# azmyrajab/polars_ols

Hardware: AMD Instinct MI355X
Metric: group_regressions_per_sec (higher is better)
Workload: dtype f32

## Files before the change

### polars_ols_amd/csrc/k4x_inverse.hip

```cpp
#include "k4_rolling.hpp"

namespace pols {

constexpr int KX_MAX = 128;

template <typename T>
struct XCtx {
    const K4Args &a;
    int64_t s;
    int first_chunk;
    int K, LD, NS, tid;
    double *P, *xs, *v, *bv, *beta, *red;
    const T *mycol;
    __device__ XCtx(const K4Args &a_, int64_t s_, int fc, double *lds) : a(a_), s(s_), first_chunk(fc) {
        K = a.k; LD = K | 1; NS = K * K + K; tid = threadIdx.x;
        P = lds; xs = P + (size_t)K * LD; v = xs + KX_MAX + 2; bv = v + KX_MAX; beta = bv + KX_MAX; red = beta + KX_MAX;
        mycol = tid < K ? static_cast<const T *>(a.xtab ? a.xtab[tid] : a.x[tid]) : static_cast<const T *>(a.y);
    }
    static __host__ __device__ size_t lds_doubles(int K) { return (size_t)K * (K | 1) + 4 * KX_MAX + 2 + 16; }

    __device__ __forceinline__ bool valid(int64_t i) const { return a.valid ? a.valid[s + i] != 0 : true; }
    __device__ __forceinline__ int64_t cnt(int64_t i) const { return a.cnt ? (int64_t)a.cnt[s + i] : i + 1; }
    __device__ __forceinline__ int64_t vidx(int64_t r) const { return a.vidx ? (int64_t)a.vidx[s + r] : r; }

    __device__ __forceinline__ void load_row(int64_t i) const {
        __syncthreads();
        if (tid <= K) xs[tid] = (double)mycol[s + i];
        __syncthreads();
    }
    __device__ double block_sum(double x) const {
        const double w = wave_sum_row3(x);
        __syncthreads();
        if ((tid & 63) == 63) red[tid >> 6] = w;
        __syncthreads();
        return red[0] + red[1] + red[2] + red[3];
    }
    __device__ void zero() const {
        for (int q = tid; q < K * LD; q += 256) P[q] = 0.0;
        if (tid < K) bv[tid] = 0.0;
        __syncthreads();
    }
    __device__ void gram_axpy(const double *src, double sign) const {
        for (int q = tid; q < K * K; q += 256) { const int i = q / K, c = q - i * K; P[i * LD + c] += sign * src[q]; }
        if (tid < K) bv[tid] += sign * src[K * K + tid];
        __syncthreads();
    }
    __device__ void gram_add_row(int64_t i, double sign) const {
        load_row(i);
        for (int q = tid; q < K * K; q += 256) { const int r = q / K, c = q - r * K; P[r * LD + c] += sign * (xs[r] * xs[c]); }
        if (tid < K) bv[tid] += sign * (xs[tid] * xs[K]);
        __syncthreads();
    }
    __device__ void gram_prefix(int64_t i, double sign, int nacc) const {
        if (i < 0) return;
        const int64_t c = i / a.chunk_len;
        gram_axpy(a.totals + (size_t)(first_chunk + c) * nacc, sign);
        for (int64_t j = c * a.chunk_len; j <= i; ++j)
            if (valid(j)) gram_add_row(j, sign);
    }
    __device__ void invert(double alpha) const {
        if (tid < K) P[tid * LD + tid] += alpha;
        __syncthreads();
        for (int j = 0; j < K; ++j) {
            const double p = 1.0 / P[j * LD + j];
            if (tid < K) v[tid] = P[tid * LD + j];
            __syncthreads();
            for (int q = tid; q < K * K; q += 256) {
                const int i = q / K, c = q - i * K;
                double val;
                if (i == j && c == j) val = -p;
                else if (i == j) val = v[c] * p;
                else if (c == j) val = v[i] * p;
                else val = P[i * LD + c] - v[i] * v[c] * p;
                P[i * LD + c] = val;
            }
            __syncthreads();
        }
        for (int q = tid; q < K * K; q += 256) { const int i = q / K, c = q - i * K; P[i * LD + c] = -P[i * LD + c]; }
        __syncthreads();
    }
    __device__ void matvec(const double *x, double *out) const {
        if (tid < K) {
            double acc = 0.0;
            const double *row = P + tid * LD;
            for (int c = 0; c < K; ++c) acc += row[c] * x[c];
            out[tid] = acc;
        }
        __syncthreads();
    }
    __device__ void rank1(double coef) const {
        for (int q = tid; q < K * K; q += 256) { const int i = q / K, c = q - i * K; P[i * LD + c] += coef * (v[i] * v[c]); }
        __syncthreads();
    }
    __device__ void sm_update(double sign) const {
        matvec(xs, v);
        const double xv = block_sum(tid < K ? xs[tid] * v[tid] : 0.0);
        rank1(-sign / (1.0 + sign * xv));
        if (tid < K) bv[tid] += sign * (xs[tid] * xs[K]);
        __syncthreads();
    }
    __device__ void solve_beta() const { matvec(bv, beta); }
    __device__ void store(int64_t i, bool have, T *coef, T *pred) const {
        const int64_t row = s + i;
        const double qnan = __longlong_as_double(0x7ff8000000000000LL);
        if (coef && tid < K) coef[row * K + tid] = (T)(have ? beta[tid] : qnan);
        if (pred) {
            load_row(i);
            const double p = block_sum(tid < K ? xs[tid] * (have ? beta[tid] : qnan) : 0.0);
            if (tid == 0) pred[row] = (T)p;
        }
    }
};

template <typename T, bool RLS>
__global__ void __launch_bounds__(256) kx_totals_kernel(const K4Args a) {
    extern __shared__ double lds[];
    const int64_t c = blockIdx.x;
    const K4Chunk ch = a.chunks[c];
    const K4Group G = a.groups[ch.group];
    XCtx<T> cx(a, G.start, G.first_chunk, lds);
    const int K = cx.K, nacc = cx.NS + (RLS ? 1 : 0);
    cx.zero();
    double decay = 1.0;
    for (int64_t i = ch.t0 - G.start; i < ch.t1 - G.start; ++i)
        if (cx.valid(i)) {
            if (RLS) {
                for (int q = cx.tid; q < K * cx.LD; q += 256) cx.P[q] *= a.ff;
                if (cx.tid < K) cx.bv[cx.tid] *= a.ff;
                decay *= a.ff;
                __syncthreads();
            }
            cx.gram_add_row(i, 1.0);
        }
    double *out = a.totals + (size_t)c * nacc;
    for (int q = cx.tid; q < K * K; q += 256) { const int i = q / K, cc = q - i * K; out[q] = cx.P[i * cx.LD + cc]; }
    if (cx.tid < K) out[K * K + cx.tid] = cx.bv[cx.tid];
    if (RLS && cx.tid == 0) out[cx.NS] = decay;
}

template <typename T>
__global__ void __launch_bounds__(256) kx_rolling_walk_kernel(const K4Args a) {
    extern __shared__ double lds[];
    const int64_t c = blockIdx.x;
    const K4Chunk ch = a.chunks[c];
    const K4Group G = a.groups[ch.group];
    XCtx<T> cx(a, G.start, G.first_chunk, lds);
    const int K = cx.K, nacc = cx.NS;
    const int64_t rel0 = ch.t0 - G.start, rel1 = ch.t1 - G.start;
    const int64_t w = a.window, mpv = G.mpv;
    const bool drop = a.drop_mode != 0;
    T *coef = static_cast<T *>(a.coef);
    T *pred = static_cast<T *>(a.pred);
    const double qnan = __longlong_as_double(0x7ff8000000000000LL);

    if (G.all_nan) {
        for (int64_t i = rel0; i < rel1; ++i) {
            if (coef && cx.tid < K) coef[(G.start + i) * K + cx.tid] = (T)qnan;
            if (pred && cx.tid == 0) pred[G.start + i] = (T)qnan;
        }
        return;
    }
    const int64_t j_min = drop ? 0 : max(mpv - w, (int64_t)0);
    const int64_t c0 = drop ? cx.cnt(mpv - 1) : 0;
    const bool longwarm = drop && c0 > w;
    auto old_of = [&](int64_t i) -> int64_t {
        if (!drop) return i - w;
        const int64_t R = cx.cnt(i) - 1;
        const int64_t r = (longwarm && R - c0 < w) ? R - c0 : R - w;
        return r < 0 ? -1 : cx.vidx(r);
    };
    auto gate = [&](int64_t i) -> bool {
        const int64_t i_start = i >= w ? i - w : 0;
        return cx.cnt(i) - cx.cnt(i_start) >= G.gate_n;
    };
    auto gram_state_at = [&](int64_t i) {
        cx.zero();
        cx.gram_prefix(i, 1.0, nacc);
        const int64_t o = (i >= 0) ? old_of(i) : -1;
        if (o >= j_min && i >= mpv) {
            cx.gram_prefix(o, -1.0, nacc);
            cx.gram_prefix(j_min - 1, 1.0, nacc);
        }
        if (longwarm && i >= mpv && cx.cnt(i) - 1 - c0 >= w) {
            cx.gram_prefix(cx.vidx(c0 - 1), 1.0, nacc);
            cx.gram_prefix(cx.vidx(w - 1), -1.0, nacc);
        }
    };

    bool inverted = false, have = false;
    int64_t prev_old = (rel0 > 0 && rel0 - 1 >= mpv) ? old_of(rel0 - 1) : -1;
    if (rel0 >= mpv && rel0 > 0) {
        int64_t ip = rel0 - 1;
        if (!(drop || ip == mpv - 1 || gate(ip))) {
            for (ip = rel0 - 2; ip >= mpv - 1; --ip)
                if (ip == mpv - 1 || gate(ip)) break;
        }
        gram_state_at(ip);
        cx.invert(a.alpha);
        cx.solve_beta();
        have = true;
        if (ip != rel0 - 1) {
            gram_state_at(rel0 - 1);
            cx.invert(a.alpha);
        }
        inverted = true;
    } else {
        gram_state_at(rel0 - 1);
    }
    for (int64_t i = rel0; i < rel1; ++i) {
        const bool vld = cx.valid(i);
        if (vld) {
            if (inverted) { cx.load_row(i); cx.sm_update(1.0); }
            else cx.gram_add_row(i, 1.0);
        }
        if (i >= mpv && (vld || !drop)) {
            const int64_t no = old_of(i);
            bool sub = false;
            if (drop) sub = (no != prev_old && no >= 0);
            else sub = (no >= j_min && no >= 0 && cx.valid(no));
            if (sub) { cx.load_row(no); cx.sm_update(-1.0); }
            prev_old = no;
        }
        if (i >= mpv - 1) {
            const bool do_solve = (i == mpv - 1) || (drop ? vld : gate(i));
            if (do_solve) {
                if (!inverted) { cx.invert(a.alpha); inverted = true; }
                cx.solve_beta();
                have = true;
            }
        }
        cx.store(i, have, coef, pred);
    }
}

template <typename T>
__global__ void __launch_bounds__(256) kx_rls_walk_kernel(const K4Args a) {
    extern __shared__ double lds[];
    const int64_t c = blockIdx.x;
    const K4Chunk ch = a.chunks[c];
    const K4Group G = a.groups[ch.group];
    XCtx<T> cx(a, G.start, G.first_chunk, lds);
    const int K = cx.K, nacc = cx.NS + 1;
    const int64_t rel0 = ch.t0 - G.start, rel1 = ch.t1 - G.start;
    T *coef = static_cast<T *>(a.coef);
    T *pred = static_cast<T *>(a.pred);
    cx.zero();
    cx.gram_axpy(a.totals + (size_t)c * nacc, 1.0);
    cx.invert(0.0);
    cx.solve_beta();
    const double ff = a.ff;
    for (int64_t i = rel0; i < rel1; ++i) {
        if (cx.valid(i)) {
            cx.load_row(i);
            cx.matvec(cx.xs, cx.v);
            const double xv = cx.block_sum(cx.tid < K ? cx.xs[cx.tid] * cx.v[cx.tid] : 0.0);
            const double xb = cx.block_sum(cx.tid < K ? cx.xs[cx.tid] * cx.beta[cx.tid] : 0.0);
            const double r = 1.0 + xv / ff;
            const double err = cx.xs[K] - xb;
            if (cx.tid < K) cx.beta[cx.tid] += cx.v[cx.tid] / (r * ff) * err;
            const double coef_vv = -1.0 / (r * ff);
            for (int q = cx.tid; q < K * K; q += 256) {
                const int ii = q / K, cc = q - ii * K;
                cx.P[ii * cx.LD + cc] = (cx.P[ii * cx.LD + cc] + coef_vv * (cx.v[ii] * cx.v[cc])) / ff;
            }
            __syncthreads();
        }
        cx.store(i, true, coef, pred);
    }
}

template <typename T>
static int kx_launch_t(pols_ctx *ctx, const K4Args &a, bool rls) {
    const size_t lds = sizeof(double) * XCtx<T>::lds_doubles(a.k);
    const int ns = a.k * a.k + a.k;
    static OncePerDevice attr_once;
    if (attr_once.needed(ctx->device)) {
        const void *fns[4] = {reinterpret_cast<const void *>(&kx_totals_kernel<T, false>), reinterpret_cast<const void *>(&kx_totals_kernel<T, true>),
                              reinterpret_cast<const void *>(&kx_rolling_walk_kernel<T>), reinterpret_cast<const void *>(&kx_rls_walk_kernel<T>)};
        for (const void *f : fns) POLS_HIP(hipFuncSetAttribute(f, hipFuncAttributeMaxDynamicSharedMemorySize, 144 * 1024));
        attr_once.done(ctx->device);
    }
    timing_begin(ctx);
    if (rls) {
        hipLaunchKernelGGL((kx_totals_kernel<T, true>), dim3((unsigned)a.n_chunks), dim3(256), lds, ctx->stream, a);
        chunk_scan_launch(ctx, a, ns, 2);
        hipLaunchKernelGGL((kx_rls_walk_kernel<T>), dim3((unsigned)a.n_chunks), dim3(256), lds, ctx->stream, a);
    } else {
        hipLaunchKernelGGL((kx_totals_kernel<T, false>), dim3((unsigned)a.n_chunks), dim3(256), lds, ctx->stream, a);
        chunk_scan_launch(ctx, a, ns, 0);
        hipLaunchKernelGGL((kx_rolling_walk_kernel<T>), dim3((unsigned)a.n_chunks), dim3(256), lds, ctx->stream, a);
    }
    timing_end(ctx);
    POLS_HIP(hipGetLastError());
    return POLS_OK;
}

int k4x_launch(pols_ctx *ctx, int dtype, const K4Args &a) {
    if (a.k > KX_MAX) return fail(POLS_ERR_UNSUPPORTED, "rolling: %d features > %d", a.k, KX_MAX);
    ctx->last_kernel = dtype == POLS_F32 ? "k4x_rolling_inverse_f32" : "k4x_rolling_inverse_f64";
    return dtype == POLS_F32 ? kx_launch_t<float>(ctx, a, false) : kx_launch_t<double>(ctx, a, false);
}

int k3x_launch(pols_ctx *ctx, int dtype, const K4Args &a) {
    if (a.k > KX_MAX) return fail(POLS_ERR_UNSUPPORTED, "rls: %d features > %d", a.k, KX_MAX);
    ctx->last_kernel = dtype == POLS_F32 ? "k3x_rls_inverse_f32" : "k3x_rls_inverse_f64";
    return dtype == POLS_F32 ? kx_launch_t<float>(ctx, a, true) : kx_launch_t<double>(ctx, a, true);
}

}
```

Before: 129.3 million.

## Prefetch rows into registers, keep beta in registers, and retile LDS element loops

Adds an 8-row register prefetch ring (XAhead) so input rows and validity flags are loaded ahead of use, replacing the per-row global load with its two barriers. Beta stays in per-thread registers instead of LDS. Element-wise matrix updates are retiled so each thread owns a column and walks rows in unrolled groups, which removes the per-element integer divide. The change also drops or merges several __syncthreads, fuses the two block reductions in RLS, and uses fma. The risks are higher register pressure, changed rounding from fma (fp contract is turned off, so only the explicit fma calls change), and subtle barrier-ordering hazards such as the double-buffered red slots used by store.

```diff
diff --git a/polars_ols_amd/csrc/k4x_inverse.hip b/polars_ols_amd/csrc/k4x_inverse.hip
--- a/polars_ols_amd/csrc/k4x_inverse.hip
+++ b/polars_ols_amd/csrc/k4x_inverse.hip
@@ -1,8 +1,33 @@
 #include "k4_rolling.hpp"
 
+#include <utility>
+
+#pragma clang fp contract(off)
+
 namespace pols {
 
 constexpr int KX_MAX = 128;
+constexpr int KX_AHEAD = 8;
+
+template <typename F, int... I>
+__device__ __forceinline__ void kx_slots(F &&f, std::integer_sequence<int, I...>) { (f(std::integral_constant<int, I>{}), ...); }
+template <typename F>
+__device__ __forceinline__ void kx_each_slot(F &&f) { kx_slots(f, std::make_integer_sequence<int, KX_AHEAD>{}); }
+
+template <typename T>
+struct XAhead {
+    T cur[KX_AHEAD], nxt[KX_AHEAD];
+    uint8_t nok[KX_AHEAD];
+    unsigned ok;
+    __device__ __forceinline__ T value(int r) const {
+        T x = cur[0];
+        kx_each_slot([&](auto j) { if (j > 0) x = (r == j) ? cur[j] : x; });
+        return x;
+    }
+    __device__ __forceinline__ bool valid(int r) const { return (ok >> r) & 1u; }
+};
+
+constexpr int KX_GROUP = 8;
 
 template <typename T>
 struct XCtx {
@@ -10,104 +35,145 @@
     int64_t s;
     int first_chunk;
     int K, LD, NS, tid;
-    double *P, *xs, *v, *bv, *beta, *red;
+    double *P, *xs, *v, *bv, *red;
     const T *mycol;
     __device__ XCtx(const K4Args &a_, int64_t s_, int fc, double *lds) : a(a_), s(s_), first_chunk(fc) {
         K = a.k; LD = K | 1; NS = K * K + K; tid = threadIdx.x;
-        P = lds; xs = P + (size_t)K * LD; v = xs + KX_MAX + 2; bv = v + KX_MAX; beta = bv + KX_MAX; red = beta + KX_MAX;
+        P = lds; xs = P + (size_t)K * LD; v = xs + KX_MAX + 2; bv = v + KX_MAX; red = bv + KX_MAX;
         mycol = tid < K ? static_cast<const T *>(a.xtab ? a.xtab[tid] : a.x[tid]) : static_cast<const T *>(a.y);
     }
-    static __host__ __device__ size_t lds_doubles(int K) { return (size_t)K * (K | 1) + 4 * KX_MAX + 2 + 16; }
+    static __host__ __device__ size_t lds_doubles(int K) { return (size_t)K * (K | 1) + 3 * KX_MAX + 2 + 16; }
 
     __device__ __forceinline__ bool valid(int64_t i) const { return a.valid ? a.valid[s + i] != 0 : true; }
     __device__ __forceinline__ int64_t cnt(int64_t i) const { return a.cnt ? (int64_t)a.cnt[s + i] : i + 1; }
     __device__ __forceinline__ int64_t vidx(int64_t r) const { return a.vidx ? (int64_t)a.vidx[s + r] : r; }
 
-    __device__ __forceinline__ void load_row(int64_t i) const {
-        __syncthreads();
-        if (tid <= K) xs[tid] = (double)mycol[s + i];
-        __syncthreads();
-    }
-    __device__ double block_sum(double x) const {
-        const double w = wave_sum_row3(x);
-        __syncthreads();
-        if ((tid & 63) == 63) red[tid >> 6] = w;
-        __syncthreads();
-        return red[0] + red[1] + red[2] + red[3];
-    }
-    __device__ void zero() const {
+    template <bool ROW, bool COL, bool EXTRA, typename F>
+    __device__ __forceinline__ void each_element(const double *rowv, const double *colv, const double *extra, F &&f) const {
+        const int wv = tid >> 6;
+        for (int c = tid & 63; c < K; c += 64) {
+            const double cv = COL ? colv[c] : 0.0;
+            int i = wv;
+            for (; i + 4 * (KX_GROUP - 1) < K; i += 4 * KX_GROUP) {
+                double pv[KX_GROUP], rv[KX_GROUP], ev[KX_GROUP];
+#pragma unroll
+                for (int u = 0; u < KX_GROUP; ++u) {
+                    const int r = i + 4 * u;
+                    pv[u] = P[r * LD + c];
+                    rv[u] = ROW ? rowv[r] : 0.0;
+                    ev[u] = EXTRA ? extra[r * K + c] : 0.0;
+                }
+#pragma unroll
+                for (int u = 0; u < KX_GROUP; ++u) {
+                    const int r = i + 4 * u;
+                    P[r * LD + c] = f(pv[u], rv[u], cv, ev[u], r, c);
+                }
+            }
+            for (; i < K; i += 4) P[i * LD + c] = f(P[i * LD + c], ROW ? rowv[i] : 0.0, cv, EXTRA ? extra[i * K + c] : 0.0, i, c);
+        }
+    }
+    __device__ __forceinline__ void ahead_fetch(XAhead<T> &h, int64_t j, int64_t lo, int64_t hi) const {
+        kx_each_slot([&](auto r) {
+            const int64_t jj = s + min(max(j + r, lo), hi);
+            h.nxt[r] = tid <= K ? mycol[jj] : T(0);
+            h.nok[r] = a.valid ? a.valid[jj] : (uint8_t)1;
+        });
+    }
+    __device__ __forceinline__ void ahead_turn(XAhead<T> &h) const {
+        h.ok = 0u;
+        kx_each_slot([&](auto r) { h.cur[r] = h.nxt[r]; h.ok |= (h.nok[r] != 0 ? 1u : 0u) << r; });
+    }
+    __device__ __forceinline__ void ahead_start(XAhead<T> &h, int64_t j, int64_t lo, int64_t hi) const {
+        ahead_fetch(h, j, lo, hi);
+        ahead_turn(h);
+        ahead_fetch(h, j + KX_AHEAD, lo, hi);
+    }
+    __device__ __forceinline__ int ahead_step(XAhead<T> &h, int64_t n, int64_t j, int64_t lo, int64_t hi) const {
+        const int r = (int)(n & (KX_AHEAD - 1));
+        if (r == 0 && n > 0) { ahead_turn(h); ahead_fetch(h, j + n + KX_AHEAD, lo, hi); }
+        return r;
+    }
+    __device__ __forceinline__ void put_row(T x) const {
+        if (tid <= K) xs[tid] = (double)x;
+        __syncthreads();
+    }
+    __device__ __forceinline__ void zero() const {
         for (int q = tid; q < K * LD; q += 256) P[q] = 0.0;
         if (tid < K) bv[tid] = 0.0;
         __syncthreads();
     }
-    __device__ void gram_axpy(const double *src, double sign) const {
-        for (int q = tid; q < K * K; q += 256) { const int i = q / K, c = q - i * K; P[i * LD + c] += sign * src[q]; }
-        if (tid < K) bv[tid] += sign * src[K * K + tid];
-        __syncthreads();
-    }
-    __device__ void gram_add_row(int64_t i, double sign) const {
-        load_row(i);
-        for (int q = tid; q < K * K; q += 256) { const int r = q / K, c = q - r * K; P[r * LD + c] += sign * (xs[r] * xs[c]); }
-        if (tid < K) bv[tid] += sign * (xs[tid] * xs[K]);
-        __syncthreads();
-    }
-    __device__ void gram_prefix(int64_t i, double sign, int nacc) const {
+    __device__ __forceinline__ void gram_axpy(const double *src, double sign) const {
+        each_element<false, false, true>(nullptr, nullptr, src, [&](double pv, double, double, double ev, int, int) { return pv + sign * ev; });
+        if (tid < K) bv[tid] = bv[tid] + sign * src[K * K + tid];
+        __syncthreads();
+    }
+    __device__ __forceinline__ void gram_add_xs(double sign) const {
+        each_element<true, true, false>(xs, xs, nullptr, [&](double pv, double xr, double xc, double, int, int) { return fma(sign * xr, xc, pv); });
+        if (tid < K) bv[tid] = fma(sign * xs[tid], xs[K], bv[tid]);
+        __syncthreads();
+    }
+    __device__ __forceinline__ void gram_prefix(int64_t i, double sign, int nacc) const {
         if (i < 0) return;
         const int64_t c = i / a.chunk_len;
         gram_axpy(a.totals + (size_t)(first_chunk + c) * nacc, sign);
-        for (int64_t j = c * a.chunk_len; j <= i; ++j)
-            if (valid(j)) gram_add_row(j, sign);
-    }
-    __device__ void invert(double alpha) const {
+        const int64_t lo = c * a.chunk_len;
+        XAhead<T> h;
+        ahead_start(h, lo, lo, i);
+        for (int64_t j = lo; j <= i; ++j) {
+            const int r = ahead_step(h, j - lo, lo, lo, i);
+            if (h.valid(r)) {
+                put_row(h.value(r));
+                gram_add_xs(sign);
+            }
+        }
+    }
+    __device__ __forceinline__ void invert(double alpha) const {
         if (tid < K) P[tid * LD + tid] += alpha;
         __syncthreads();
         for (int j = 0; j < K; ++j) {
             const double p = 1.0 / P[j * LD + j];
             if (tid < K) v[tid] = P[tid * LD + j];
             __syncthreads();
-            for (int q = tid; q < K * K; q += 256) {
-                const int i = q / K, c = q - i * K;
-                double val;
-                if (i == j && c == j) val = -p;
-                else if (i == j) val = v[c] * p;
-                else if (c == j) val = v[i] * p;
-                else val = P[i * LD + c] - v[i] * v[c] * p;
-                P[i * LD + c] = val;
-            }
-            __syncthreads();
-        }
-        for (int q = tid; q < K * K; q += 256) { const int i = q / K, c = q - i * K; P[i * LD + c] = -P[i * LD + c]; }
-        __syncthreads();
-    }
-    __device__ void matvec(const double *x, double *out) const {
+            each_element<true, true, false>(v, v, nullptr, [&](double pv, double vi, double vc, double, int i, int c) {
+                return i == j ? (c == j ? -p : vc * p) : (c == j ? vi * p : fma(-p, vi * vc, pv));
+            });
+            __syncthreads();
+        }
+        each_element<false, false, false>(nullptr, nullptr, nullptr, [&](double pv, double, double, double, int, int) { return -pv; });
+        __syncthreads();
+    }
+    __device__ __forceinline__ double matvec(const double *x) const {
+        double acc = 0.0;
         if (tid < K) {
-            double acc = 0.0;
             const double *row = P + tid * LD;
-            for (int c = 0; c < K; ++c) acc += row[c] * x[c];
-            out[tid] = acc;
-        }
-        __syncthreads();
-    }
-    __device__ void rank1(double coef) const {
-        for (int q = tid; q < K * K; q += 256) { const int i = q / K, c = q - i * K; P[i * LD + c] += coef * (v[i] * v[c]); }
-        __syncthreads();
-    }
-    __device__ void sm_update(double sign) const {
-        matvec(xs, v);
-        const double xv = block_sum(tid < K ? xs[tid] * v[tid] : 0.0);
-        rank1(-sign / (1.0 + sign * xv));
-        if (tid < K) bv[tid] += sign * (xs[tid] * xs[K]);
-        __syncthreads();
-    }
-    __device__ void solve_beta() const { matvec(bv, beta); }
-    __device__ void store(int64_t i, bool have, T *coef, T *pred) const {
-        const int64_t row = s + i;
+#pragma unroll 16
+            for (int c = 0; c < K; ++c) acc = fma(row[c], x[c], acc);
+        }
+        return acc;
+    }
+    __device__ __forceinline__ void sm_update(double sign) const {
+        const double vt = matvec(xs);
+        if (tid < K) v[tid] = vt;
+        const double w = wave_sum_row3(tid < K ? xs[tid] * vt : 0.0);
+        if ((tid & 63) == 63) red[tid >> 6] = w;
+        __syncthreads();
+        const double xv = red[0] + red[1] + red[2] + red[3];
+        const double coef = -sign / (1.0 + sign * xv);
+        each_element<true, true, false>(v, v, nullptr, [&](double pv, double vi, double vc, double, int, int) { return fma(coef, vi * vc, pv); });
+        if (tid < K) bv[tid] = fma(sign * xs[tid], xs[K], bv[tid]);
+        __syncthreads();
+    }
+    __device__ __forceinline__ void store(int64_t row, bool have, double bt, T x, int slot, T *coef, T *pred, bool always_sync) const {
         const double qnan = __longlong_as_double(0x7ff8000000000000LL);
-        if (coef && tid < K) coef[row * K + tid] = (T)(have ? beta[tid] : qnan);
+        if (coef && tid < K) coef[row * K + tid] = (T)(have ? bt : qnan);
         if (pred) {
-            load_row(i);
-            const double p = block_sum(tid < K ? xs[tid] * (have ? beta[tid] : qnan) : 0.0);
-            if (tid == 0) pred[row] = (T)p;
+            const double w = wave_sum_row3(tid < K ? (double)x * (have ? bt : qnan) : 0.0);
+            double *rd = red + 8 + 4 * slot;
+            if ((tid & 63) == 63) rd[tid >> 6] = w;
+            __syncthreads();
+            if (tid == 0) pred[row] = (T)(rd[0] + rd[1] + rd[2] + rd[3]);
+        } else if (always_sync) {
+            __syncthreads();
         }
     }
 };
@@ -120,20 +186,30 @@
     const K4Group G = a.groups[ch.group];
     XCtx<T> cx(a, G.start, G.first_chunk, lds);
     const int K = cx.K, nacc = cx.NS + (RLS ? 1 : 0);
+    const int64_t rel0 = ch.t0 - G.start, rel1 = ch.t1 - G.start;
+    const double ff = a.ff;
     cx.zero();
     double decay = 1.0;
-    for (int64_t i = ch.t0 - G.start; i < ch.t1 - G.start; ++i)
-        if (cx.valid(i)) {
+    if (rel1 > rel0) {
+        XAhead<T> h;
+        cx.ahead_start(h, rel0, rel0, rel1 - 1);
+        for (int64_t i = rel0; i < rel1; ++i) {
+            const int r = cx.ahead_step(h, i - rel0, rel0, rel0, rel1 - 1);
+            if (!h.valid(r)) continue;
+            cx.put_row(h.value(r));
             if (RLS) {
-                for (int q = cx.tid; q < K * cx.LD; q += 256) cx.P[q] *= a.ff;
-                if (cx.tid < K) cx.bv[cx.tid] *= a.ff;
-                decay *= a.ff;
+                cx.template each_element<true, true, false>(cx.xs, cx.xs, nullptr, [&](double pv, double xr, double xc, double, int, int) { return fma(xr, xc, pv * ff); });
+                if (cx.tid < K) cx.bv[cx.tid] = fma(cx.xs[cx.tid], cx.xs[K], cx.bv[cx.tid] * ff);
+                decay *= ff;
                 __syncthreads();
+            } else {
+                cx.gram_add_xs(1.0);
             }
-            cx.gram_add_row(i, 1.0);
-        }
+        }
+    }
     double *out = a.totals + (size_t)c * nacc;
-    for (int q = cx.tid; q < K * K; q += 256) { const int i = q / K, cc = q - i * K; out[q] = cx.P[i * cx.LD + cc]; }
+    for (int c2 = cx.tid & 63; c2 < K; c2 += 64)
+        for (int i = cx.tid >> 6; i < K; i += 4) out[i * K + c2] = cx.P[i * cx.LD + c2];
     if (cx.tid < K) out[K * K + cx.tid] = cx.bv[cx.tid];
     if (RLS && cx.tid == 0) out[cx.NS] = decay;
 }
@@ -160,6 +236,7 @@
         }
         return;
     }
+    if (rel1 <= rel0) return;
     const int64_t j_min = drop ? 0 : max(mpv - w, (int64_t)0);
     const int64_t c0 = drop ? cx.cnt(mpv - 1) : 0;
     const bool longwarm = drop && c0 > w;
@@ -175,61 +252,79 @@
     };
     auto gram_state_at = [&](int64_t i) {
         cx.zero();
-        cx.gram_prefix(i, 1.0, nacc);
         const int64_t o = (i >= 0) ? old_of(i) : -1;
-        if (o >= j_min && i >= mpv) {
-            cx.gram_prefix(o, -1.0, nacc);
-            cx.gram_prefix(j_min - 1, 1.0, nacc);
-        }
-        if (longwarm && i >= mpv && cx.cnt(i) - 1 - c0 >= w) {
-            cx.gram_prefix(cx.vidx(c0 - 1), 1.0, nacc);
-            cx.gram_prefix(cx.vidx(w - 1), -1.0, nacc);
+        const bool slid = o >= j_min && i >= mpv;
+        const bool kept = longwarm && i >= mpv && cx.cnt(i) - 1 - c0 >= w;
+#pragma nounroll
+        for (int t = 0; t < 5; ++t) {
+            int64_t upto = -1;
+            if (t == 0) upto = i;
+            else if (t == 1 && slid) upto = o;
+            else if (t == 2 && slid) upto = j_min - 1;
+            else if (t == 3 && kept) upto = cx.vidx(c0 - 1);
+            else if (t == 4 && kept) upto = cx.vidx(w - 1);
+            cx.gram_prefix(upto, (t == 1 || t == 4) ? -1.0 : 1.0, nacc);
         }
     };
 
     bool inverted = false, have = false;
+    double bt = 0.0;
     int64_t prev_old = (rel0 > 0 && rel0 - 1 >= mpv) ? old_of(rel0 - 1) : -1;
-    if (rel0 >= mpv && rel0 > 0) {
-        int64_t ip = rel0 - 1;
-        if (!(drop || ip == mpv - 1 || gate(ip))) {
-            for (ip = rel0 - 2; ip >= mpv - 1; --ip)
-                if (ip == mpv - 1 || gate(ip)) break;
-        }
-        gram_state_at(ip);
-        cx.invert(a.alpha);
-        cx.solve_beta();
-        have = true;
-        if (ip != rel0 - 1) {
-            gram_state_at(rel0 - 1);
+    const bool carry = rel0 >= mpv && rel0 > 0;
+    int64_t ip = rel0 - 1;
+    if (carry && !(drop || ip == mpv - 1 || gate(ip))) {
+        for (ip = rel0 - 2; ip >= mpv - 1; --ip)
+            if (ip == mpv - 1 || gate(ip)) break;
+    }
+#pragma nounroll
+    for (int pass = 0; pass < 2; ++pass) {
+        if (pass == 1) {
+            if (ip == rel0 - 1) break;
+            __syncthreads();
+        }
+        gram_state_at(pass == 0 ? ip : rel0 - 1);
+        if (carry) {
             cx.invert(a.alpha);
-        }
-        inverted = true;
-    } else {
-        gram_state_at(rel0 - 1);
-    }
+            inverted = true;
+            if (pass == 0) { bt = cx.matvec(cx.bv); have = true; }
+        }
+    }
+    const bool out_ahead = a.vidx == nullptr;
+    const int64_t hi = rel1 - 1;
+    XAhead<T> in, out;
+    cx.ahead_start(in, rel0, rel0, hi);
+    if (out_ahead) cx.ahead_start(out, rel0 - w, 0, hi);
     for (int64_t i = rel0; i < rel1; ++i) {
-        const bool vld = cx.valid(i);
+        const int r = cx.ahead_step(in, i - rel0, rel0, rel0, hi);
+        if (out_ahead) cx.ahead_step(out, i - rel0, rel0 - w, 0, hi);
+        const T xi = in.value(r);
+        const bool vld = in.valid(r);
         if (vld) {
-            if (inverted) { cx.load_row(i); cx.sm_update(1.0); }
-            else cx.gram_add_row(i, 1.0);
+            cx.put_row(xi);
+            if (inverted) cx.sm_update(1.0);
+            else cx.gram_add_xs(1.0);
         }
         if (i >= mpv && (vld || !drop)) {
             const int64_t no = old_of(i);
+            const bool near = out_ahead && no == i - w;
             bool sub = false;
             if (drop) sub = (no != prev_old && no >= 0);
-            else sub = (no >= j_min && no >= 0 && cx.valid(no));
-            if (sub) { cx.load_row(no); cx.sm_update(-1.0); }
+            else sub = (no >= j_min && no >= 0 && (near ? out.valid(r) : cx.valid(no)));
+            if (sub) {
+                cx.put_row(near ? out.value(r) : (cx.tid <= K ? cx.mycol[cx.s + no] : T(0)));
+                cx.sm_update(-1.0);
+            }
             prev_old = no;
         }
         if (i >= mpv - 1) {
             const bool do_solve = (i == mpv - 1) || (drop ? vld : gate(i));
             if (do_solve) {
                 if (!inverted) { cx.invert(a.alpha); inverted = true; }
-                cx.solve_beta();
+                bt = cx.matvec(cx.bv);
                 have = true;
             }
         }
-        cx.store(i, have, coef, pred);
+        cx.store(G.start + i, have, bt, xi, (int)(i & 1), coef, pred, false);
     }
 }
 
@@ -240,32 +335,41 @@
     const K4Chunk ch = a.chunks[c];
     const K4Group G = a.groups[ch.group];
     XCtx<T> cx(a, G.start, G.first_chunk, lds);
-    const int K = cx.K, nacc = cx.NS + 1;
+    const int K = cx.K, nacc = cx.NS + 1, tid = cx.tid;
     const int64_t rel0 = ch.t0 - G.start, rel1 = ch.t1 - G.start;
     T *coef = static_cast<T *>(a.coef);
     T *pred = static_cast<T *>(a.pred);
+    if (rel1 <= rel0) return;
     cx.zero();
     cx.gram_axpy(a.totals + (size_t)c * nacc, 1.0);
     cx.invert(0.0);
-    cx.solve_beta();
+    double bt = cx.matvec(cx.bv);
     const double ff = a.ff;
+    const int64_t hi = rel1 - 1;
+    XAhead<T> h;
+    cx.ahead_start(h, rel0, rel0, hi);
     for (int64_t i = rel0; i < rel1; ++i) {
-        if (cx.valid(i)) {
-            cx.load_row(i);
-            cx.matvec(cx.xs, cx.v);
-            const double xv = cx.block_sum(cx.tid < K ? cx.xs[cx.tid] * cx.v[cx.tid] : 0.0);
-            const double xb = cx.block_sum(cx.tid < K ? cx.xs[cx.tid] * cx.beta[cx.tid] : 0.0);
-            const double r = 1.0 + xv / ff;
+        const int r = cx.ahead_step(h, i - rel0, rel0, rel0, hi);
+        const T xi = h.value(r);
+        if (h.valid(r)) {
+            const double xd = (double)xi;
+            cx.put_row(xi);
+            const double vt = cx.matvec(cx.xs);
+            if (tid < K) cx.v[tid] = vt;
+            const double wv = wave_sum_row3(tid < K ? xd * vt : 0.0);
+            const double wb = wave_sum_row3(tid < K ? xd * bt : 0.0);
+            if ((tid & 63) == 63) { cx.red[tid >> 6] = wv; cx.red[4 + (tid >> 6)] = wb; }
+            __syncthreads();
+            const double xv = cx.red[0] + cx.red[1] + cx.red[2] + cx.red[3];
+            const double xb = cx.red[4] + cx.red[5] + cx.red[6] + cx.red[7];
+            const double rr = 1.0 + xv / ff;
             const double err = cx.xs[K] - xb;
-            if (cx.tid < K) cx.beta[cx.tid] += cx.v[cx.tid] / (r * ff) * err;
-            const double coef_vv = -1.0 / (r * ff);
-            for (int q = cx.tid; q < K * K; q += 256) {
-                const int ii = q / K, cc = q - ii * K;
-                cx.P[ii * cx.LD + cc] = (cx.P[ii * cx.LD + cc] + coef_vv * (cx.v[ii] * cx.v[cc])) / ff;
-            }
-            __syncthreads();
-        }
-        cx.store(i, true, coef, pred);
+            const double rf = rr * ff;
+            if (tid < K) bt = fma(vt / rf, err, bt);
+            const double coef_vv = -1.0 / rf;
+            cx.template each_element<true, true, false>(cx.v, cx.v, nullptr, [&](double pv, double vi, double vc, double, int, int) { return fma(coef_vv, vi * vc, pv) / ff; });
+        }
+        cx.store(G.start + i, true, bt, xi, (int)(i & 1), coef, pred, true);
     }
 }
 
```

Result: no change. 129.7 million (median of 3 runs) (+0.3%).
